# valerio98-lab/DQL_multirotor_landing

Measured on NVIDIA B200. Metric: env_steps_per_sec_incl_q_updates, higher is better.
Workload: dtype f32

## Files before the change

### dql_multirotor_landing_b200/csrc/env_state.cuh

```cuda
#pragma once
#include "dqlb200_device.cuh"

namespace dql {


constexpr int CELLS = DQLB200_MAX_CELLS;
constexpr uint32_t FULL = 0xFFFFFFFFu;

__device__ __forceinline__ uint4 lds128(unsigned addr) {
  uint4 v;
  asm volatile("ld.shared.v4.u32 {%0, %1, %2, %3}, [%4];" : "=r"(v.x), "=r"(v.y), "=r"(v.z), "=r"(v.w) : "r"(addr) : "memory");
  return v;
}

constexpr uint32_t SID_BITS = 10, STEP_SHIFT = 10, STEP_BITS = 9, CC_SHIFT = 19, CC_BITS = 5;
constexpr uint32_t STICKY_BIT = 1u << 24, FRESH_BIT = 1u << 25, BP_SHIFT = 26;

struct Env {
  Body b;
  uint32_t sp_idx;
  float prev_rel_p, prev_rel_v;
  uint32_t sid, bp, step_count, curriculum_check;
  bool sticky_success, fresh;
  uint32_t episode;
  double cum_reward;
};

constexpr size_t ENV_TILE_BYTES = 3 * 32 * 16;
struct EnvPtrs {
  unsigned char* base;
  int n_p, tiles_per_pop;
  uint4* d;
  uint4* e;
  size_t n;
  const double* sp_value;
  const uint2* sp_next;
  const double* sp_rtheta;
  int sp_zero, n_sp;
};
__device__ __forceinline__ unsigned char* env_addr(const EnvPtrs& p, int pop, int env) {
  return p.base + ((size_t)pop * p.tiles_per_pop + (size_t)(env >> 5)) * ENV_TILE_BYTES + (size_t)(env & 31) * 16;
}
__device__ __forceinline__ unsigned char* env_addr(const EnvPtrs& p, size_t i) {
  const int pop = (int)(i / (size_t)p.n_p);
  return env_addr(p, pop, (int)(i - (size_t)pop * p.n_p));
}
__device__ __forceinline__ Ext ext_load(const EnvPtrs& p, size_t i) {
  const uint4 u = p.e[i], v = p.e[p.n + i];
  return Ext{__uint_as_float(u.x), __uint_as_float(u.y), __uint_as_float(u.z), __uint_as_float(u.w),
             __uint_as_float(v.x), __uint_as_float(v.y), __uint_as_float(v.z), __uint_as_float(v.w)};
}
__device__ __forceinline__ void ext_store(const EnvPtrs& p, size_t i, const Ext& x) {
  p.e[i] = make_uint4(__float_as_uint(x.omega), __float_as_uint(x.z), __float_as_uint(x.v_z), __float_as_uint(x.integ));
  p.e[p.n + i] = make_uint4(__float_as_uint(x.e1), __float_as_uint(x.f1), __float_as_uint(x.f2), __float_as_uint(x.f3));
}
template <class KT>
__device__ __forceinline__ Ext ext_initial(const KT& kc) { return Ext{0.0f, kc.z_init, 0.0f, kc.pid_i0, 0.0f, 0.0f, 0.0f, 0.0f}; }
__device__ __forceinline__ Kf kf_load(const EnvPtrs& p, size_t i) {
  const uint4 v = p.d[i];
  return Kf{__uint_as_float(v.x), __uint_as_float(v.y), __uint_as_float(v.z), v.w};
}
__device__ __forceinline__ void kf_store(const EnvPtrs& p, size_t i, const Kf& f) {
  p.d[i] = make_uint4(__float_as_uint(f.x), __float_as_uint(f.P), __float_as_uint(f.v_ref), f.n);
}
__device__ __forceinline__ void ext_prefetch_async(const EnvPtrs& p, size_t i, unsigned stage_addr, int nt, bool filt, bool so) {
  if (filt) asm volatile("cp.async.cg.shared.global [%0], [%1], 16;" ::"r"(stage_addr), "l"(p.d + i) : "memory");
  if (so) {
    asm volatile("cp.async.cg.shared.global [%0], [%1], 16;" ::"r"(stage_addr + 16u * nt), "l"(p.e + i) : "memory");
    asm volatile("cp.async.cg.shared.global [%0], [%1], 16;" ::"r"(stage_addr + 32u * nt), "l"(p.e + p.n + i) : "memory");
  }
  asm volatile("cp.async.commit_group;" ::: "memory");
}
__device__ __forceinline__ Kf kf_take(unsigned stage_addr, int nt) {
  asm volatile("cp.async.wait_group 0;" ::: "memory");
  const uint4 v = lds128(stage_addr);
  return Kf{__uint_as_float(v.x), __uint_as_float(v.y), __uint_as_float(v.z), v.w};
}
__device__ __forceinline__ Ext ext_take(unsigned stage_addr, int nt) {
  asm volatile("cp.async.wait_group 0;" ::: "memory");
  const uint4 u = lds128(stage_addr + 16u * nt), v = lds128(stage_addr + 32u * nt);
  return Ext{__uint_as_float(u.x), __uint_as_float(u.y), __uint_as_float(u.z), __uint_as_float(u.w),
             __uint_as_float(v.x), __uint_as_float(v.y), __uint_as_float(v.z), __uint_as_float(v.w)};
}
__device__ __forceinline__ Kf kf_initial() { return Kf{0.0f, 1.0f, 0.0f, 0u}; }

struct EnvRaw {
  float4 A;
  uint4 B, C;
};
__device__ __forceinline__ EnvRaw env_fetch(const unsigned char* pa) {
  EnvRaw r;
  r.A = __ldcg(reinterpret_cast<const float4*>(pa));
  r.B = __ldcg(reinterpret_cast<const uint4*>(pa + 512));
  r.C = __ldcg(reinterpret_cast<const uint4*>(pa + 1024));
  return r;
}
__device__ __forceinline__ void tile_mbar_init(unsigned mbar) {
  asm volatile("mbarrier.init.shared::cta.b64 [%0], 1;" ::"r"(mbar) : "memory");
  asm volatile("fence.mbarrier_init.release.cluster;" ::: "memory");
  asm volatile("fence.proxy.async.shared::cta;" ::: "memory");
}
__device__ __forceinline__ void tile_prefetch_bulk(const unsigned char* tile, unsigned stage_tile, unsigned mbar) {
  asm volatile("mbarrier.arrive.expect_tx.shared::cta.b64 _, [%0], %1;" ::"r"(mbar), "n"((int)ENV_TILE_BYTES) : "memory");
  asm volatile("cp.async.bulk.shared::cluster.global.mbarrier::complete_tx::bytes [%0], [%1], %2, [%3];" ::"r"(stage_tile), "l"(tile),
               "n"((int)ENV_TILE_BYTES), "r"(mbar)
               : "memory");
}
__device__ __forceinline__ void tile_wait(unsigned mbar, uint32_t parity) {
  asm volatile(
      "{\n"
      ".reg .pred p;\n"
      "TILE_WAIT:\n"
      "mbarrier.try_wait.parity.shared::cta.b64 p, [%0], %1;\n"
      "@p bra TILE_DONE;\n"
      "bra TILE_WAIT;\n"
      "TILE_DONE:\n"
      "}\n" ::"r"(mbar),
      "r"(parity)
      : "memory");
}
__device__ __forceinline__ EnvRaw tile_take(unsigned stage_lane) {
  EnvRaw r;
  const uint4 a = lds128(stage_lane);
  r.A = make_float4(__uint_as_float(a.x), __uint_as_float(a.y), __uint_as_float(a.z), __uint_as_float(a.w));
  r.B = lds128(stage_lane + 512u);
  r.C = lds128(stage_lane + 1024u);
  return r;
}

__device__ __forceinline__ void env_unpack(const EnvRaw& r, Env& e) {
  const float4 A = r.A;
  const uint4 B = r.B;
  const uint4 Cw = r.C;
  e.b.x_d = A.x; e.b.v_d = A.y; e.b.theta = A.z; e.b.phase = __float_as_uint(A.w); e.b.a_d = 0.0f;
  e.sp_idx = B.x;
  e.prev_rel_p = __uint_as_float(B.z);
  e.prev_rel_v = __uint_as_float(B.w);
  e.sid = Cw.x & ((1u << SID_BITS) - 1u);
  e.step_count = (Cw.x >> STEP_SHIFT) & ((1u << STEP_BITS) - 1u);
  e.curriculum_check = (Cw.x >> CC_SHIFT) & ((1u << CC_BITS) - 1u);
  e.sticky_success = (Cw.x & STICKY_BIT) != 0u;
  e.bp = (Cw.x >> BP_SHIFT) & 3u;
  e.fresh = (Cw.x & FRESH_BIT) != 0u;
  e.episode = Cw.y;
  e.cum_reward = __hiloint2double((int)Cw.w, (int)Cw.z);
}
__device__ __forceinline__ void env_store(unsigned char* pa, const Env& e) {
  __stcg(reinterpret_cast<float4*>(pa), make_float4(e.b.x_d, e.b.v_d, e.b.theta, __uint_as_float(e.b.phase)));
  __stcg(reinterpret_cast<uint4*>(pa + 512), make_uint4(e.sp_idx, 0u, __float_as_uint(e.prev_rel_p), __float_as_uint(e.prev_rel_v)));
  const uint32_t packed = e.sid | (e.step_count << STEP_SHIFT) | (e.curriculum_check << CC_SHIFT) |
                          (e.sticky_success ? STICKY_BIT : 0u) | (e.fresh ? FRESH_BIT : 0u) | (e.bp << BP_SHIFT);
  __stcg(reinterpret_cast<uint4*>(pa + 1024), make_uint4(packed, e.episode, (uint32_t)__double2loint(e.cum_reward),
                                                          (uint32_t)__double2hiint(e.cum_reward)));
}
__device__ __forceinline__ void env_load(const EnvPtrs& p, size_t i, Env& e) { env_unpack(env_fetch(env_addr(p, i)), e); }
__device__ __forceinline__ void env_store(const EnvPtrs& p, size_t i, const Env& e) { env_store(env_addr(p, i), e); }

template <class KT, class AC>
__device__ __forceinline__ void env_reset(const KT& kc, const dqlb200_population_params& pp,
                                          const dqlb200_cuts& cuts, const AC& angle_cut, Env& e,
                                          uint32_t env_index, uint32_t birth, int w, bool fresh_mdp, uint32_t sp_zero, Kf* kf = nullptr, Ext* ext = nullptr) {
  const uint4 d = philox4x32_10(make_uint4(env_index, birth, PURPOSE_RESET, pp.population_id), pp.seed_lo, pp.seed_hi);
  Obs o = dyn_reset(kc, pp, e.b, d, w == 0, false, kc.dz_train, kf, ext);
  if (kc.noise_enabled) {
    const uint4 dn = philox4x32_10(make_uint4(env_index, birth, PURPOSE_RESET_NOISE, pp.population_id), pp.seed_lo, pp.seed_hi);
    add_observation_noise(kc, o, dn.x, dn.y);
  }
  const DState ds0 = discretise_cuts(cuts, angle_cut, o);
  e.sid = (uint32_t)ds0.id();
  e.bp = (uint32_t)ds0.bp;
  e.step_count = 0;
  e.curriculum_check = 0;
  e.sticky_success = false;
  e.fresh = true;
  e.cum_reward = 0.0;
  if (fresh_mdp) {
    e.sp_idx = sp_zero;
    e.prev_rel_p = 0.0f;
    e.prev_rel_v = 0.0f;
    e.episode = 0;
  }
}


}
```

### dql_multirotor_landing_b200/csrc/train_kernel.cuh

```cuda
#pragma once
#include <type_traits>

#include "env_state.cuh"

namespace dql {

#define DQL_BAR_CASE(OP, ID) case (ID - 1): if (WARPS >= ID) asm volatile("barrier." OP " " #ID ", 64;" ::: "memory"); break;
template <int WARPS>
__device__ __forceinline__ void baton_wait(int warp) {
  switch (warp) {
    DQL_BAR_CASE("sync", 1) DQL_BAR_CASE("sync", 2) DQL_BAR_CASE("sync", 3) DQL_BAR_CASE("sync", 4)
    DQL_BAR_CASE("sync", 5) DQL_BAR_CASE("sync", 6) DQL_BAR_CASE("sync", 7) DQL_BAR_CASE("sync", 8)
    default: break;
  }
}
template <int WARPS>
__device__ __forceinline__ void baton_pass(int next_warp) {
  switch (next_warp) {
    DQL_BAR_CASE("arrive", 1) DQL_BAR_CASE("arrive", 2) DQL_BAR_CASE("arrive", 3) DQL_BAR_CASE("arrive", 4)
    DQL_BAR_CASE("arrive", 5) DQL_BAR_CASE("arrive", 6) DQL_BAR_CASE("arrive", 7) DQL_BAR_CASE("arrive", 8)
    default: break;
  }
}
#undef DQL_BAR_CASE

#ifdef DQL_TIMING
__device__ unsigned long long dql_timing[4096 * 8];
#define DQL_STAMP(i)                                                                                                      \
  do {                                                                                                                    \
    if (threadIdx.x == 0 && blockIdx.x < 2048) {                                                                          \
      unsigned long long t_;                                                                                              \
      asm volatile("mov.u64 %0, %%globaltimer;" : "=l"(t_)::"memory");                                                    \
      dql_timing[blockIdx.x * 8 + (i)] = t_;                                                                              \
    }                                                                                                                     \
  } while (0)
#else
#define DQL_STAMP(i) do { } while (0)
#endif

struct TrainArgs {
  EnvPtrs env;
  uint32_t* tables;
  dqlb200_population_state* pop_state;
  const dqlb200_population_params* pop_params;
  const float* alpha_luts;
  const uint32_t* eps_threshold;
  dqlb200_trace trace;
  uint32_t* merge_snapshot;
  int k_steps;
  int pop_offset;
  long long n_total;
};

constexpr int RESET_QUEUE = 64;

constexpr int STATES = DQLB200_MAX_CURRICULUM * DQLB200_STATES_PER_LEVEL;

constexpr int EP_OK_CAP = 128;
constexpr int EP_RET_CAP = 32;

struct Shared {
  float qa[CELLS];
  uint32_t cnt[CELLS];
  float qmax[STATES];
  uint8_t greedy[STATES + 3];
  dqlb200_cuts cuts;
  dqlb200_reward_level reward[DQLB200_MAX_CURRICULUM];
  dqlb200_population_state ps;
  uint32_t step_episodes, step_success, step_ep_steps, step_hist[9];
  int promote, advance, do_advance;
  uint4 philox_keys[5];
  double ep_ret[EP_RET_CAP];
  uint8_t ep_ok[EP_OK_CAP];
  int n_ep_ok, n_ep_ret;
};

struct SpEntry {
  uint32_t next;
  float value;
  double r_step, r_first;
};
__host__ __device__ constexpr size_t train_sp_bytes(int n_setpoints) { return ((size_t)n_setpoints * 3 * sizeof(SpEntry) + 15) & ~size_t(15); }
__host__ __device__ constexpr size_t train_smem_bytes(int threads, bool extended, int n_setpoints) {
  return ((sizeof(Shared) + 15) & ~size_t(15)) + train_sp_bytes(n_setpoints) + (size_t)(threads / 32) * RESET_QUEUE * sizeof(uint16_t) +
         (size_t)(extended ? 6 : 3) * threads * 16 + (((size_t)(threads / 32) * 8 + 15) & ~size_t(15));
}

static_assert((train_smem_bytes(128, false, 33) + 1024) * 6 <= 228 * 1024, "train_kernel<4>: six CTAs per SM no longer fit in shared memory");
#ifndef DQL_WARPS_PER_SM
#define DQL_WARPS_PER_SM 24
#endif
#ifndef DQL_WARPS_PER_SM_GENERIC
#define DQL_WARPS_PER_SM_GENERIC 20
#endif
template <bool GENERIC_> struct ConstsOf;
template <> struct ConstsOf<true> {
  __device__ __forceinline__ static const KC& get(const KC& kc) { return kc; }
};
template <> struct ConstsOf<false> {
  __device__ __forceinline__ static KDef get(const KC&) { return KDef{}; }
};

template <int WARPS, bool TRACE, int VARIANT>
__global__ void __launch_bounds__(WARPS * 32, ((VARIANT == 2 ? DQL_WARPS_PER_SM_GENERIC : DQL_WARPS_PER_SM) / WARPS) > 0 ? ((VARIANT == 2 ? DQL_WARPS_PER_SM_GENERIC : DQL_WARPS_PER_SM) / WARPS) : 1) train_kernel(const __grid_constant__ KC kc, const TrainArgs args) {
  constexpr bool GENERIC = VARIANT == 1 || VARIANT == 2, EXT = VARIANT == 2, FULL_SLOTS = VARIANT == 3;
  extern __shared__ __align__(16) unsigned char smem_raw[];
  Shared& sh = *reinterpret_cast<Shared*>(smem_raw);
  DQL_STAMP(0);
#ifdef DQL_TIMING
  if (threadIdx.x == 0 && blockIdx.x < 2048) {
    unsigned smid_, warpid_;
    asm volatile("mov.u32 %0, %%smid;" : "=r"(smid_));
    asm volatile("mov.u32 %0, %%warpid;" : "=r"(warpid_));
    dql_timing[4096 * 8 - 1 - blockIdx.x] = ((unsigned long long)smid_ << 32) | warpid_;
  }
#endif
  const auto& kk = ConstsOf<GENERIC>::get(kc);
  const int tid = threadIdx.x, lane = tid & 31, warp = tid >> 5;
  constexpr int NT = WARPS * 32;
  const int pop = blockIdx.x + args.pop_offset;
  const int n_p = kc.envs_per_population;
  const int n_slots = (n_p + NT - 1) / NT;
  unsigned char* dyn = smem_raw + ((sizeof(Shared) + 15) & ~size_t(15));
  uint16_t* reset_queue = reinterpret_cast<uint16_t*>(dyn) + (size_t)warp * RESET_QUEUE;
  dyn += (size_t)WARPS * RESET_QUEUE * sizeof(uint16_t);
  uint4* stage = reinterpret_cast<uint4*>(dyn);
  dyn += (size_t)((TRACE || EXT) ? 6 : 3) * NT * 16;
  unsigned long long* tile_mbar = reinterpret_cast<unsigned long long*>(dyn);
  dyn += ((size_t)WARPS * 8 + 15) & ~size_t(15);
  SpEntry* sp_tab = reinterpret_cast<SpEntry*>(dyn);
  const unsigned stage_tile = (unsigned)__cvta_generic_to_shared(stage) + (unsigned)warp * (unsigned)ENV_TILE_BYTES;
  const unsigned stage_lane = stage_tile + (unsigned)lane * 16u;
  const unsigned ext_stage = (unsigned)__cvta_generic_to_shared(stage + WARPS * 96 + tid);
  const unsigned mbar = (unsigned)__cvta_generic_to_shared(tile_mbar + warp);
  const int tiles_pp = args.env.tiles_per_pop;
  uint32_t tile_phase = 0u;
  bool tile_pending = false;
  auto prefetch_tile = [&](const unsigned char* tile) {
    __syncwarp();
    if (lane == 0) tile_prefetch_bulk(tile, stage_tile, mbar);
    tile_pending = true;
  };
  auto env_writes_done = [&]() { asm volatile("fence.proxy.async.global;" ::: "memory"); };
  auto wait_tile = [&]() {
    tile_wait(mbar, tile_phase);
    tile_phase ^= 1u;
    tile_pending = false;
  };
  const size_t env_base = (size_t)pop * n_p;
  uint32_t* gt = args.tables + (size_t)pop * 3 * CELLS;
  float* gqb = reinterpret_cast<float*>(gt + CELLS);
  const uint32_t sp_zero = (uint32_t)args.env.sp_zero;

  static_assert(sizeof(dqlb200_population_state) % 4 == 0, "word copies");
  constexpr int PS_WORDS = sizeof(dqlb200_population_state) / 4;
  const dqlb200_population_params pp = args.pop_params[pop];
  unsigned char* const p_tile0 = env_addr(args.env, pop, warp * 32);
  if (lane == 0) tile_mbar_init(mbar);
  if (warp < tiles_pp) prefetch_tile(p_tile0);
  if (EXT) ext_prefetch_async(args.env, env_base + (size_t)min(tid, n_p - 1), ext_stage, NT, kc.accel_mode != 0, kc.dynamics_model != 0);
  {
    const int w_start = args.pop_state[pop].working_step;
    const uint32_t* gps = reinterpret_cast<const uint32_t*>(args.pop_state + pop);
    for (int i = tid; i < PS_WORDS; i += NT) reinterpret_cast<uint32_t*>(&sh.ps)[i] = gps[i];
    if (tid == 0) {
      sh.step_episodes = sh.step_success = sh.step_ep_steps = 0u;
      for (int i = 0; i < 9; ++i) sh.step_hist[i] = 0u;
      sh.promote = sh.advance = sh.do_advance = 0;
      sh.n_ep_ok = sh.n_ep_ret = 0;
      sh.cuts = kc.cuts[w_start];
    }
    if (tid < 5) sh.reward[tid] = kc.reward[tid];
    if (tid == 31) philox_round_keys(pp.seed_lo, pp.seed_hi, sh.philox_keys);
    for (int i = tid; i < args.env.n_sp * 3; i += NT) {
      const uint2 nx = args.env.sp_next[i];
      sp_tab[i] = SpEntry{nx.x, __uint_as_float(nx.y), args.env.sp_rtheta[i], args.env.sp_rtheta[DQLB200_MAX_SETPOINTS * 3 + i]};
    }
    const int live = (w_start + 1) * DQLB200_CELLS_PER_LEVEL;
    for (int i = tid; i < DQLB200_CELLS_PER_LEVEL; i += NT) {
      sh.qa[i] = __uint_as_float(gt[i]);
      sh.cnt[i] = gt[2 * CELLS + i];
      if ((i & 31) == 0) asm volatile("prefetch.global.L2 [%0];" ::"l"(gqb + i));
    }
    for (int i = DQLB200_CELLS_PER_LEVEL + tid; i < live; i += NT) {
      sh.qa[i] = __uint_as_float(gt[i]);
      sh.cnt[i] = gt[2 * CELLS + i];
      if ((i & 31) == 0) asm volatile("prefetch.global.L2 [%0];" ::"l"(gqb + i));
    }
  }
  __syncthreads();

  DQL_STAMP(1);
  const float* __restrict__ alpha_lut = args.alpha_luts + (size_t)pp.alpha_lut * DQLB200_ALPHA_LUT;
  const float alpha_min = __ldg(alpha_lut + DQLB200_ALPHA_LUT - 1);
  const bool filt = EXT && kc.accel_mode != 0;
  const bool so = EXT && kc.dynamics_model != 0;
  uint64_t steps_done = 0;

  auto build_snapshot = [&](int w) {
    for (int st = tid; st < (w + 1) * DQLB200_STATES_PER_LEVEL; st += NT) {
      const float q0 = sh.qa[st * 3 + 0], q1 = sh.qa[st * 3 + 1], q2 = sh.qa[st * 3 + 2];
      const float p0 = fmul(fadd(q0, __ldcg(gqb + st * 3 + 0)), 0.5f);
      const float p1 = fmul(fadd(q1, __ldcg(gqb + st * 3 + 1)), 0.5f);
      const float p2 = fmul(fadd(q2, __ldcg(gqb + st * 3 + 2)), 0.5f);
      int a = 0;
      float best = p0;
      if (p1 > best) { best = p1; a = 1; }
      if (p2 > best) { a = 2; }
      sh.greedy[st] = (uint8_t)a;
      sh.qmax[st] = fmaxf(fmaxf(q0, q1), q2);
    }
  };

  auto drain_episode_log = [&]() {
    dqlb200_population_state& ps = sh.ps;
    const int n_fin = sh.n_ep_ok, n_ret = sh.n_ep_ret;
    if (n_fin == 0) return;
    const int L = kc.window_len;
    bool promote = false;
    if (lane == 31) {
      double s = ps.return_sum;
      for (int i = 0; i < n_ret; ++i) s = __dadd_rn(s, sh.ep_ret[i]);
      ps.return_sum = s;
    }
    for (int base = 0; base < n_fin; base += 32) {
      const int n = min(32, n_fin - base);
      const bool mine = lane < n;
      const int ok = mine ? (int)sh.ep_ok[base + lane] : 0;
      const uint32_t smask = __ballot_sync(FULL, ok != 0);
      const int head = ps.window_head, count = ps.window_count, sum = ps.window_sum;
      if (n <= L) {
        int pos = head + lane;
        pos -= (pos >= L) ? L : 0;
        const bool evicts = mine && (count + lane >= L);
        const int old = evicts ? (int)ps.window[pos] : 0;
        const uint32_t emask = __ballot_sync(FULL, evicts && old != 0);
        const uint32_t upto = (2u << lane) - 1u;
        const int s_here = sum + __popc(smask & upto) - __popc(emask & upto);
        promote = promote || __any_sync(FULL, mine && s_here >= kc.promote_successes);
        __syncwarp();
        if (mine) ps.window[pos] = (uint8_t)ok;
        if (lane == 0) {
          int h2 = head + n;
          h2 -= (h2 >= L) ? L : 0;
          ps.window_head = h2;
          ps.window_count = min(count + n, L);
          ps.window_sum = sum + __popc(smask) - __popc(emask);
        }
      } else {
        bool pr = false;
        if (lane == 0) {
          int h2 = head, c2 = count, s2 = sum;
          for (int b = 0; b < n; ++b) {
            const int okb = (smask >> b) & 1u;
            if (c2 == L) s2 -= ps.window[h2];
            else c2 += 1;
            ps.window[h2] = (uint8_t)okb;
            s2 += okb;
            h2 = (h2 + 1 == L) ? 0 : h2 + 1;
            pr = pr || (s2 >= kc.promote_successes);
          }
          ps.window_head = h2; ps.window_count = c2; ps.window_sum = s2;
        }
        promote = promote || (__shfl_sync(FULL, (int)pr, 0) != 0);
      }
      __syncwarp();
    }
    if (lane == 0) {
      ps.episodes_in_step += n_fin;
      if (kc.replicas == 1) {
        if (promote) sh.promote = 1;
        if (ps.episodes_in_step >= kc.max_num_episodes) sh.advance = 1;
      }
      sh.n_ep_ok = sh.n_ep_ret = 0;
    }
    __syncwarp();
  };

  auto advance_curriculum = [&](int w, uint32_t birth) {
    const int cs = kc.curriculum_steps;
    int dst = -1, src = 0;
    float ratio = 1.0f;
    if (kc.transfer_mode == 0) { dst = w; src = (w - 1 + cs) % cs; ratio = kc.transfer_ratio[w]; }
    else if (w + 1 < cs) { dst = w + 1; src = w; ratio = kc.transfer_ratio[w + 1]; }
    if (dst >= 0) {
      uint32_t* sg = (args.merge_snapshot && pop % kc.replicas == 0) ? args.merge_snapshot + (size_t)(pop / kc.replicas) * 3 * CELLS : nullptr;
      for (int i = tid; i < DQLB200_CELLS_PER_LEVEL; i += NT) {
        const float q_src = (src <= w) ? sh.qa[src * DQLB200_CELLS_PER_LEVEL + i] : __uint_as_float(gt[src * DQLB200_CELLS_PER_LEVEL + i]);
        const float qa_new = fmul(q_src, ratio), qb_new = fmul(gqb[src * DQLB200_CELLS_PER_LEVEL + i], ratio);
        sh.qa[dst * DQLB200_CELLS_PER_LEVEL + i] = qa_new;
        gqb[dst * DQLB200_CELLS_PER_LEVEL + i] = qb_new;
        if (sg) {
          sg[dst * DQLB200_CELLS_PER_LEVEL + i] = __float_as_uint(qa_new);
          sg[CELLS + dst * DQLB200_CELLS_PER_LEVEL + i] = __float_as_uint(qb_new);
        }
      }
    }
    if (w + 1 < cs) {
      for (int i = tid; i < DQLB200_CELLS_PER_LEVEL; i += NT) {
        const int c = (w + 1) * DQLB200_CELLS_PER_LEVEL + i;
        if (dst != w + 1) sh.qa[c] = __uint_as_float(gt[c]);
        sh.cnt[c] = gt[2 * CELLS + c];
      }
    }
    __syncthreads();
    if (tid == 0) {
      dqlb200_population_state& ps = sh.ps;
      if (sh.promote) { ps.window_head = ps.window_count = ps.window_sum = 0; }
      ps.promoted_at[w] = birth;
      ps.episodes_in_step = 0;
      ps.pending_advance = 0;
      sh.promote = sh.advance = sh.do_advance = 0;
      if (w + 1 >= cs) ps.finished = 1;
      else {
        ps.working_step = w + 1;
        sh.cuts = kc.cuts[w + 1];
      }
    }
    __syncthreads();
    if (!sh.ps.finished) {
      for (int slot = 0; slot < n_slots; ++slot) {
        const int env_i = slot * NT + tid;
        if (env_i < n_p) {
          Env e;
          Kf kf;
          Ext ex;
          if (filt) kf = kf_load(args.env, env_base + env_i);
          if (so) ex = ext_load(args.env, env_base + env_i);
          env_reset(kk, pp, sh.cuts, kk.angle_cut, e, (uint32_t)env_i, birth, w + 1, true, sp_zero, filt ? &kf : nullptr, so ? &ex : nullptr);
          env_store(env_addr(args.env, pop, env_i), e);
          if (filt) kf_store(args.env, env_base + env_i, kf);
          if (so) ext_store(args.env, env_base + env_i, ex);
        }
      }
      env_writes_done();
      if (tile_pending) wait_tile();
      if (warp < tiles_pp) prefetch_tile(p_tile0);
      if (EXT) {
        asm volatile("cp.async.wait_group 0;" ::: "memory");
        ext_prefetch_async(args.env, env_base + (size_t)min(tid, n_p - 1), ext_stage, NT, filt, so);
      }
      build_snapshot(w + 1);
    }
    __syncthreads();
  };
  if (sh.ps.pending_advance && !sh.ps.finished) {
    if (tid == 0) sh.promote = (sh.ps.pending_advance == 1) ? 1 : 0;
    __syncthreads();
    advance_curriculum(sh.ps.working_step, sh.ps.t);
  } else {
    build_snapshot(sh.ps.working_step);
    __syncthreads();
  }

  DQL_STAMP(2);
  for (int k = 0; k < args.k_steps; ++k) {
    if (sh.ps.finished) break;
    const int w = sh.ps.working_step;
    const uint32_t t = sh.ps.t;
    int n_queued = 0;

    auto flush_resets = [&]() {
      __syncwarp();
      for (int base = 0; base < n_queued; base += 32) {
        if (base + lane < n_queued) {
          const int qv = reset_queue[base + lane];
          const int env_r = (qv >> 5) * NT + warp * 32 + (qv & 31);
          const size_t gr = env_base + (size_t)env_r;
          unsigned char* const pr = env_addr(args.env, pop, env_r);
          Env e;
          env_unpack(env_fetch(pr), e);
          Kf kf;
          Ext ex;
          if (filt) kf = kf_load(args.env, gr);
          if (so) ex = ext_load(args.env, gr);
          env_reset(kk, pp, sh.cuts, kk.angle_cut, e, (uint32_t)env_r, t + 1u, w, false, sp_zero, filt ? &kf : nullptr, so ? &ex : nullptr);
          env_store(pr, e);
          if (filt) kf_store(args.env, gr, kf);
          if (so) ext_store(args.env, gr, ex);
        }
      }
      __syncwarp();
      n_queued = 0;
    };

    auto slot_loop = [&](auto w0_tag) {
    constexpr bool W0 = decltype(w0_tag)::value;
    bool bad_obs = false;
    unsigned char* p_env = env_addr(args.env, pop, tid);
    for (int slot = 0; slot < n_slots; ++slot) {
      const int env_i = slot * NT + tid;
      const bool valid = FULL_SLOTS || env_i < n_p;
      const size_t gi = env_base + (size_t)env_i;
      if (FULL_SLOTS || slot * WARPS + warp < tiles_pp) wait_tile();
      if (slot == 0) DQL_STAMP(7);
      const EnvRaw cur_raw = tile_take(stage_lane);
      unsigned char* const p_cur = p_env;
      p_env += WARPS * ENV_TILE_BYTES;
      Kf kf;
      Ext ex;
      if (filt) kf = kf_take(ext_stage, NT);
      if (so) ex = ext_take(ext_stage, NT);
      if (FULL_SLOTS ? (slot + 1 < n_slots) : ((slot + 1) * WARPS + warp < tiles_pp)) prefetch_tile(p_env - (size_t)lane * 16);
      if (EXT && env_i + NT < n_p) ext_prefetch_async(args.env, gi + NT, ext_stage, NT, filt, so);
      uint32_t cell = 0;
      float target = 0.0f;
      bool done = false, success = false;
      int code = 0;
      uint32_t ep_steps = 0;
      double ep_return = 0.0;
      Env e;
      int a = 0;
      uint32_t sid = 0u, noise_w0 = 0u, noise_w1 = 0u;
      size_t trace_i = 0;
      if (valid) {
        env_unpack(cur_raw, e);
        sid = e.sid;
        a = sh.greedy[sid];
        if (W0 || w == 0 || (GENERIC && kk.noise_enabled)) {
          const uint4 d = philox4x32_10_keyed(make_uint4((uint32_t)env_i, t, PURPOSE_STEP, pp.population_id), sh.philox_keys);
          if (W0 || w == 0) {
            const uint32_t thr = __ldg(args.eps_threshold + min(e.episode, (uint32_t)(DQLB200_EPS_LUT - 1)));
            if ((d.x >> 8) < thr) a = (int)__umulhi(d.y, 3u);
          }
          if (GENERIC) { noise_w0 = d.z; noise_w1 = d.w; }
        }
        if (TRACE) {
          trace_i = (size_t)k * (size_t)args.n_total + gi;
          if (args.trace.action_override) {
            const int o = args.trace.action_override[trace_i];
            if (o >= 0) a = o;
          }
        }
        cell = sid * 3u + (uint32_t)a;
      }
      uint32_t peers;
      asm volatile("match.any.sync.b32 %0, %1, 0xffffffff;" : "=r"(peers) : "r"(valid ? cell : (0x80000000u | (uint32_t)lane)) : "memory");
      uint2 spn = make_uint2(0u, 0u);
      double r_theta0 = 0.0;
      Obs o = {};
      DState ds = {};
      uint32_t sid2 = 0u, step_count = 0u, cc = 0u;
      if (valid) {
        const uint32_t sp_prev = e.sp_idx;
        {
          const SpEntry* en = sp_tab + (e.fresh ? sp_zero : sp_prev) * 3u + (uint32_t)a;
          spn = make_uint2(en->next, __float_as_uint(en->value));
        }
        const float sp = __uint_as_float(spn.y);
        r_theta0 = *(&sp_tab[sp_prev * 3u + (uint32_t)a].r_step + (e.fresh ? 1 : 0));
        dyn_advance(kk, pp, e.b, sp, filt ? &kf : nullptr, so ? &ex : nullptr, kk.vz_train);
        step_count = e.step_count + 1u;
        o = dyn_observe(kk, pp, e.b, (int)step_count, kk.dz_train, filt ? &kf : nullptr, so ? &ex : nullptr);
        if (GENERIC && kk.noise_enabled) add_observation_noise(kk, o, noise_w0, noise_w1);
        ds = W0 ? discretise_cuts(kc.cuts[0], kk.angle_cut, o, 0) : discretise_cuts(sh.cuts, kk.angle_cut, o, w);
        sid2 = (uint32_t)ds.id();
        const bool t_fx = !(o.rel_p >= kk.fz_lo) || (o.rel_p >= kk.fz_hi);
        const bool t_zmin = !(o.z >= kk.z_min_cut), t_zmax = o.z >= kk.z_max_cut;
        const bool t_time = (int)step_count >= kk.timeout_steps;
        const bool goal_bins = !(o.contact || t_fx || t_zmin || t_zmax || t_time) && ds.bp == 1 && ds.bv == 1;
        const bool at_level = W0 || (sid >= (uint32_t)(w * DQLB200_STATES_PER_LEVEL) && ds.level == w);
        cc = goal_bins ? (at_level ? e.curriculum_check + 1u : 0u) : e.curriculum_check;
        code = e.sticky_success ? DQLB200_NON_TERMINAL_SUCCESS : DQLB200_NON_TERMINAL;
        if (goal_bins && at_level) code = ((int)cc >= kk.success_steps) ? DQLB200_TERMINAL_SUCCESS : DQLB200_NON_TERMINAL_SUCCESS;
        code = t_time ? DQLB200_TERMINAL_TIMEOUT : code;
        code = t_zmax ? DQLB200_TERMINAL_FLYZONE_Z : code;
        code = t_zmin ? DQLB200_TERMINAL_MINIMUM_ALTITUDE : code;
        code = t_fx ? DQLB200_TERMINAL_FLYZONE_X : code;
        code = o.contact ? DQLB200_TERMINAL_CONTACT : code;
        done = code >= DQLB200_TERMINAL_SUCCESS;
        success = code == DQLB200_TERMINAL_SUCCESS;
        bad_obs = bad_obs || !(fabsf(o.rel_p) <= 3.4028234664e38f) || !(fabsf(o.rel_v) <= 3.4028234664e38f) || !(fabsf(o.rel_a) <= 3.4028234664e38f);
      }
      const uint32_t lower = peers & ((1u << lane) - 1u);
      const int rank = __popc(lower);
      const int n_group = valid ? __popc(peers) : 0;
      const int pred = lower ? (31 - __clz(lower)) : lane;
      const bool is_last = valid && (peers >> lane) == 1u;
      const int n_max = __reduce_max_sync(FULL, n_group);
      const uint32_t c_hint = min(sh.cnt[cell] + (uint32_t)rank, (uint32_t)(DQLB200_ALPHA_LUT - 1));
      const float a_hint = __ldg(alpha_lut + c_hint);
      if (valid) {
        const double phi_p = shaping(kk.w_p, o.rel_p, kk.p_max, kk.rcp_p_max, kk.clip_p_f, GENERIC);
        const double phi_v = shaping(kk.w_v, o.rel_v, kk.v_max, kk.rcp_v_max, kk.clip_v_f, GENERIC);
        const double prev_p = shaping(kk.w_p, e.prev_rel_p, kk.p_max, kk.rcp_p_max, kk.clip_p_f, GENERIC);
        const double prev_v = shaping(kk.w_v, e.prev_rel_v, kk.v_max, kk.rcp_v_max, kk.clip_v_f, GENERIC);
        const bool succ_reward = code == DQLB200_NON_TERMINAL_SUCCESS || code == DQLB200_TERMINAL_SUCCESS;
        const double r = reward_sp(W0 ? kc.reward[0] : sh.reward[ds.level], phi_p, phi_v, prev_p, prev_v, r_theta0, succ_reward);
        const float qn = sh.qmax[sid2];
        const float changed = (e.bp != (uint32_t)ds.bp) ? 1.0f : 0.0f;
        target = fadd((float)r, fmul(fmul(kk.gamma, qn), changed));
        if (TRACE) {
          if (args.trace.obs) {
            float* po = args.trace.obs + trace_i * 5;
            po[0] = o.rel_p; po[1] = o.rel_v; po[2] = o.rel_a; po[3] = o.pitch; po[4] = o.z;
          }
          if (args.trace.reward) args.trace.reward[trace_i] = r;
          if (args.trace.action) args.trace.action[trace_i] = (uint8_t)a;
          if (args.trace.code) args.trace.code[trace_i] = (uint8_t)code;
          if (args.trace.done) args.trace.done[trace_i] = (uint8_t)done;
          if (args.trace.contact) args.trace.contact[trace_i] = (uint8_t)o.contact;
          if (args.trace.state) args.trace.state[trace_i] = (uint16_t)sid;
          if (args.trace.next_state) args.trace.next_state[trace_i] = (uint16_t)sid2;
          if (args.trace.episode) args.trace.episode[trace_i] = (int32_t)e.episode;
        }
        ep_steps = step_count;
        ep_return = e.cum_reward;
        e.sp_idx = spn.x;
        e.prev_rel_p = o.rel_p;
        e.prev_rel_v = o.rel_v;
        e.episode += done ? 1u : 0u;
        e.sid = sid2;
        e.bp = (uint32_t)ds.bp;
        e.step_count = step_count;
        e.curriculum_check = cc;
        e.sticky_success = (code == DQLB200_NON_TERMINAL_SUCCESS);
        e.fresh = false;
        e.cum_reward = __dadd_rn(e.cum_reward, r);
      }
      const uint32_t dmask = __ballot_sync(FULL, valid && done);
      uint32_t smask = 0u;
      double ret = 0.0;
      if (dmask) {
        smask = __ballot_sync(FULL, valid && success);
        ret = (valid && done) ? ep_return : 0.0;
#pragma unroll
        for (int off = 16; off > 0; off >>= 1) ret = __dadd_rn(ret, __shfl_xor_sync(FULL, ret, off));
      }
      if (WARPS > 1 && !(slot == 0 && warp == 0)) baton_wait<WARPS>(warp);
      {
        float q = sh.qa[cell];
        const uint32_t c0 = sh.cnt[cell];
        const uint32_t c_pre = min(c0 + (uint32_t)rank, (uint32_t)(DQLB200_ALPHA_LUT - 1));
        float alpha = a_hint;
        if (c_pre != c_hint) alpha = __ldg(alpha_lut + c_pre);
        if (rank == 0) q = fadd(q, fmul(alpha, fsub(target, q)));
#pragma unroll 1
        for (int r = 1; r < n_max; ++r) {
          const float qp = __shfl_sync(FULL, q, pred);
          if (rank == r) q = fadd(qp, fmul(alpha, fsub(target, qp)));
        }
        if (is_last) {
          sh.qa[cell] = q;
          sh.cnt[cell] = c0 + (uint32_t)n_group;
        }
        if (dmask) {
          if (sh.n_ep_ret == EP_RET_CAP || sh.n_ep_ok > EP_OK_CAP - 32) drain_episode_log();
          const int idx = sh.n_ep_ret, base = sh.n_ep_ok;
          const int last = 31 - __clz(dmask);
          __syncwarp();
          if (valid && done) sh.ep_ok[base + __popc(dmask & ((1u << lane) - 1u))] = (uint8_t)success;
          if (lane == 0) {
            sh.ep_ret[idx] = ret;
            sh.n_ep_ret = idx + 1;
            sh.n_ep_ok = base + __popc(dmask);
          }
          if (lane == last) {
            sh.ps.last_cumulative = ep_return;
            sh.ps.last_steps = (int)ep_steps;
            sh.ps.last_code = code;
          }
        }
      }
      if (WARPS > 1 && !(slot == n_slots - 1 && warp == WARPS - 1)) {
        baton_pass<WARPS>((warp + 1) % WARPS);
      }
      if (dmask) {
        if (valid && done) {
          atomicAdd(&sh.step_hist[code], 1u);
          atomicAdd(&sh.step_ep_steps, ep_steps);
        }
        if (lane == 0) {
          atomicAdd(&sh.step_episodes, (uint32_t)__popc(dmask));
          atomicAdd(&sh.step_success, (uint32_t)__popc(smask));
        }
      }
      if (valid) env_store(p_cur, e);
      if (filt && valid) kf_store(args.env, gi, kf);
      if (so && valid) ext_store(args.env, gi, ex);
      if (dmask) {
        if (valid && done) reset_queue[n_queued + __popc(dmask & ((1u << lane) - 1u))] = (uint16_t)(slot * 32 + lane);
        n_queued += __popc(dmask);
        if (n_queued > RESET_QUEUE - 32) flush_resets();
      }
      if (slot == 0) DQL_STAMP(6);
    }
    if (bad_obs) atomicOr(&sh.ps.error_flags, 1u);
    };
    if constexpr (!GENERIC && !TRACE) {
      if (w == 0) slot_loop(std::true_type{});
      else slot_loop(std::false_type{});
    } else {
      slot_loop(std::false_type{});
    }
    flush_resets();
    env_writes_done();
    if (k + 1 < args.k_steps) {
      if (warp < tiles_pp) prefetch_tile(p_tile0);
      if (EXT) ext_prefetch_async(args.env, env_base + (size_t)min(tid, n_p - 1), ext_stage, NT, filt, so);
    }
    __syncthreads();
    DQL_STAMP(3);
    steps_done += (uint64_t)n_p;
    if (warp == 0) drain_episode_log();
    if (tid == 0) {
      sh.ps.t = t + 1u;
      sh.do_advance = (sh.promote || sh.advance) ? 1 : 0;
      sh.ps.total_episodes += sh.step_episodes; sh.ps.total_successes += sh.step_success; sh.ps.episode_steps_sum += sh.step_ep_steps;
      sh.step_episodes = sh.step_success = sh.step_ep_steps = 0u;
    }
    if (tid < 9) { sh.ps.termination_hist[tid] += sh.step_hist[tid]; sh.step_hist[tid] = 0u; }
    if (k + 1 < args.k_steps) build_snapshot(w);
    __syncthreads();
    if (sh.do_advance) advance_curriculum(w, t + 1u);
  }

  DQL_STAMP(4);
  if (tile_pending) wait_tile();
  if (EXT) asm volatile("cp.async.wait_all;" ::: "memory");
  for (int i = tid; i < (sh.ps.working_step + 1) * DQLB200_CELLS_PER_LEVEL; i += NT) {
    gt[i] = __float_as_uint(sh.qa[i]);
    gt[2 * CELLS + i] = sh.cnt[i];
  }
  if (warp == 0) {
    if (lane == 0) {
      dqlb200_population_state& ps = sh.ps;
      ps.total_steps += steps_done;
    }
    __syncwarp();
    uint32_t* gps = reinterpret_cast<uint32_t*>(args.pop_state + pop);
    for (int i = lane; i < PS_WORDS; i += 32) gps[i] = reinterpret_cast<const uint32_t*>(&sh.ps)[i];
  }
  DQL_STAMP(5);
}


}
```

Baseline: 28.95 billion.

## Pair consecutive env tiles per warp in stage-0 loop to halve baton handoffs

In the w==0 fast path, each warp now processes two adjacent env tiles per baton turn. The front half of the first tile is stashed in idle rows of the Q-table shared memory, and a second bulk tile prefetch lands in that scratch area. Both Q-updates are then committed under a single baton wait/pass, cutting the serialized inter-warp handoffs in half. Reset-queue indexing and tile addressing are remapped to the paired layout. The cost is more complex mbarrier expect_tx/arrive bookkeeping, reliance on unused shared table rows, and extra register/stash traffic.

```diff
diff --git a/dql_multirotor_landing_b200/csrc/env_state.cuh b/dql_multirotor_landing_b200/csrc/env_state.cuh
--- a/dql_multirotor_landing_b200/csrc/env_state.cuh
+++ b/dql_multirotor_landing_b200/csrc/env_state.cuh
@@ -106,6 +106,13 @@
                "n"((int)ENV_TILE_BYTES), "r"(mbar)
                : "memory");
 }
+__device__ __forceinline__ void tile_prefetch_bulk_noarrive(const unsigned char* tile, unsigned stage_tile, unsigned mbar) {
+  asm volatile("mbarrier.expect_tx.relaxed.cta.shared::cta.b64 [%0], %1;" ::"r"(mbar), "n"((int)ENV_TILE_BYTES) : "memory");
+  asm volatile("cp.async.bulk.shared::cluster.global.mbarrier::complete_tx::bytes [%0], [%1], %2, [%3];" ::"r"(stage_tile), "l"(tile),
+               "n"((int)ENV_TILE_BYTES), "r"(mbar)
+               : "memory");
+}
+__device__ __forceinline__ void tile_arrive(unsigned mbar) { asm volatile("mbarrier.arrive.shared::cta.b64 _, [%0];" ::"r"(mbar) : "memory"); }
 __device__ __forceinline__ void tile_wait(unsigned mbar, uint32_t parity) {
   asm volatile(
       "{\n"
diff --git a/dql_multirotor_landing_b200/csrc/train_kernel.cuh b/dql_multirotor_landing_b200/csrc/train_kernel.cuh
--- a/dql_multirotor_landing_b200/csrc/train_kernel.cuh
+++ b/dql_multirotor_landing_b200/csrc/train_kernel.cuh
@@ -1,4 +1,5 @@
 #pragma once
+#include <cstddef>
 #include <type_traits>
 
 #include "env_state.cuh"
@@ -85,6 +86,33 @@
   return ((sizeof(Shared) + 15) & ~size_t(15)) + train_sp_bytes(n_setpoints) + (size_t)(threads / 32) * RESET_QUEUE * sizeof(uint16_t) +
          (size_t)(extended ? 6 : 3) * threads * 16 + (((size_t)(threads / 32) * 8 + 15) & ~size_t(15));
 }
+
+struct PairStash {
+  uint4 lane[32];
+  uint32_t dmask, smask, n_max, last_sc;
+  double ret, last_ret;
+};
+constexpr size_t PAIR_QA = (DQLB200_CELLS_PER_LEVEL * sizeof(float) + 15) & ~size_t(15);
+constexpr size_t PAIR_CNT = (offsetof(Shared, cnt) + DQLB200_CELLS_PER_LEVEL * sizeof(uint32_t) + 15) & ~size_t(15);
+constexpr size_t PAIR_QA_END = offsetof(Shared, qa) + CELLS * sizeof(float), PAIR_CNT_END = offsetof(Shared, cnt) + CELLS * sizeof(uint32_t);
+constexpr int PAIR_TILES_IN_QA = (int)((PAIR_QA_END - PAIR_QA) / ENV_TILE_BYTES);
+__host__ __device__ constexpr size_t pair_tile_off(int warp) {
+  return warp < PAIR_TILES_IN_QA ? PAIR_QA + (size_t)warp * ENV_TILE_BYTES : PAIR_CNT + (size_t)(warp - PAIR_TILES_IN_QA) * ENV_TILE_BYTES;
+}
+__host__ __device__ constexpr size_t pair_stash_off(int warps, int warp) {
+  return PAIR_CNT + (size_t)(warps > PAIR_TILES_IN_QA ? warps - PAIR_TILES_IN_QA : 0) * ENV_TILE_BYTES + (size_t)warp * sizeof(PairStash);
+}
+static_assert(offsetof(Shared, qa) == 0 && sizeof(PairStash) % 16 == 0, "scratch offsets are 16-byte aligned");
+static_assert(PAIR_TILES_IN_QA >= 4 && pair_stash_off(8, 8) <= PAIR_CNT_END, "paired slots: second tiles and stashes of 8 warps no longer fit in the idle table rows");
+
+struct TileFront {
+  Env e;
+  uint32_t cell, c_hint, ep_steps, dmask, smask;
+  float target, a_hint;
+  int code, rank, pred, n_group, n_max;
+  bool done, is_last;
+  double ep_return, ret;
+};
 
 static_assert((train_smem_bytes(128, false, 33) + 1024) * 6 <= 228 * 1024, "train_kernel<4>: six CTAs per SM no longer fit in shared memory");
 #ifndef DQL_WARPS_PER_SM
@@ -155,12 +183,13 @@
   static_assert(sizeof(dqlb200_population_state) % 4 == 0, "word copies");
   constexpr int PS_WORDS = sizeof(dqlb200_population_state) / 4;
   const dqlb200_population_params pp = args.pop_params[pop];
-  unsigned char* const p_tile0 = env_addr(args.env, pop, warp * 32);
+  constexpr bool PAIRED_W0 = FULL_SLOTS && !GENERIC && !TRACE;
+  auto tile0 = [&](int w_) { return env_addr(args.env, pop, ((PAIRED_W0 && w_ == 0 && n_slots > 1) ? 2 * warp : warp) * 32); };
+  const int w_start = args.pop_state[pop].working_step;
   if (lane == 0) tile_mbar_init(mbar);
-  if (warp < tiles_pp) prefetch_tile(p_tile0);
+  if (warp < tiles_pp) prefetch_tile(tile0(w_start));
   if (EXT) ext_prefetch_async(args.env, env_base + (size_t)min(tid, n_p - 1), ext_stage, NT, kc.accel_mode != 0, kc.dynamics_model != 0);
   {
-    const int w_start = args.pop_state[pop].working_step;
     const uint32_t* gps = reinterpret_cast<const uint32_t*>(args.pop_state + pop);
     for (int i = tid; i < PS_WORDS; i += NT) reinterpret_cast<uint32_t*>(&sh.ps)[i] = gps[i];
     if (tid == 0) {
@@ -335,7 +364,7 @@
       }
       env_writes_done();
       if (tile_pending) wait_tile();
-      if (warp < tiles_pp) prefetch_tile(p_tile0);
+      if (warp < tiles_pp) prefetch_tile(tile0(w + 1));
       if (EXT) {
         asm volatile("cp.async.wait_group 0;" ::: "memory");
         ext_prefetch_async(args.env, env_base + (size_t)min(tid, n_p - 1), ext_stage, NT, filt, so);
@@ -360,12 +389,15 @@
     const uint32_t t = sh.ps.t;
     int n_queued = 0;
 
-    auto flush_resets = [&]() {
+    auto flush_resets = [&](auto paired_tag) {
+      constexpr bool PAIRED = decltype(paired_tag)::value;
       __syncwarp();
       for (int base = 0; base < n_queued; base += 32) {
         if (base + lane < n_queued) {
           const int qv = reset_queue[base + lane];
-          const int env_r = (qv >> 5) * NT + warp * 32 + (qv & 31);
+          const int j = qv >> 5;
+          const int env_r = (PAIRED && ((j & 1) || j + 1 < n_slots)) ? (j & ~1) * NT + (2 * warp + (j & 1)) * 32 + (qv & 31)
+                                                                      : j * NT + warp * 32 + (qv & 31);
           const size_t gr = env_base + (size_t)env_r;
           unsigned char* const pr = env_addr(args.env, pop, env_r);
           Env e;
@@ -384,32 +416,15 @@
       n_queued = 0;
     };
 
-    auto slot_loop = [&](auto w0_tag) {
-    constexpr bool W0 = decltype(w0_tag)::value;
-    bool bad_obs = false;
-    unsigned char* p_env = env_addr(args.env, pop, tid);
-    for (int slot = 0; slot < n_slots; ++slot) {
-      const int env_i = slot * NT + tid;
-      const bool valid = FULL_SLOTS || env_i < n_p;
-      const size_t gi = env_base + (size_t)env_i;
-      if (FULL_SLOTS || slot * WARPS + warp < tiles_pp) wait_tile();
-      if (slot == 0) DQL_STAMP(7);
-      const EnvRaw cur_raw = tile_take(stage_lane);
-      unsigned char* const p_cur = p_env;
-      p_env += WARPS * ENV_TILE_BYTES;
-      Kf kf;
-      Ext ex;
-      if (filt) kf = kf_take(ext_stage, NT);
-      if (so) ex = ext_take(ext_stage, NT);
-      if (FULL_SLOTS ? (slot + 1 < n_slots) : ((slot + 1) * WARPS + warp < tiles_pp)) prefetch_tile(p_env - (size_t)lane * 16);
-      if (EXT && env_i + NT < n_p) ext_prefetch_async(args.env, gi + NT, ext_stage, NT, filt, so);
+    auto tile_front = [&](auto w0_tag, TileFront& f, const EnvRaw& cur_raw, int env_i, bool valid, size_t gi, Kf& kf, Ext& ex, bool& bad_obs) {
+      constexpr bool W0 = decltype(w0_tag)::value;
       uint32_t cell = 0;
       float target = 0.0f;
       bool done = false, success = false;
       int code = 0;
       uint32_t ep_steps = 0;
       double ep_return = 0.0;
-      Env e;
+      Env& e = f.e;
       int a = 0;
       uint32_t sid = 0u, noise_w0 = 0u, noise_w1 = 0u;
       size_t trace_i = 0;
@@ -527,76 +542,172 @@
 #pragma unroll
         for (int off = 16; off > 0; off >>= 1) ret = __dadd_rn(ret, __shfl_xor_sync(FULL, ret, off));
       }
+      f.cell = cell; f.c_hint = c_hint; f.ep_steps = ep_steps; f.dmask = dmask; f.smask = smask;
+      f.target = target; f.a_hint = a_hint;
+      f.code = code; f.rank = rank; f.pred = pred; f.n_group = n_group; f.n_max = n_max;
+      f.done = done; f.is_last = is_last;
+      f.ep_return = ep_return; f.ret = ret;
+    };
+
+    auto tile_commit = [&](uint32_t cell, float target, float a_hint, uint32_t c_hint, int rank, int pred, int n_group, bool is_last, int n_max,
+                           uint32_t dmask, uint32_t smask, double ret, int writer, double last_ret, uint32_t last_steps, int last_code, bool done, bool success) {
+      float q = sh.qa[cell];
+      const uint32_t c0 = sh.cnt[cell];
+      const uint32_t c_pre = min(c0 + (uint32_t)rank, (uint32_t)(DQLB200_ALPHA_LUT - 1));
+      float alpha = a_hint;
+      if (c_pre != c_hint) alpha = __ldg(alpha_lut + c_pre);
+      if (rank == 0) q = fadd(q, fmul(alpha, fsub(target, q)));
+#pragma unroll 1
+      for (int r = 1; r < n_max; ++r) {
+        const float qp = __shfl_sync(FULL, q, pred);
+        if (rank == r) q = fadd(qp, fmul(alpha, fsub(target, qp)));
+      }
+      if (is_last) {
+        sh.qa[cell] = q;
+        sh.cnt[cell] = c0 + (uint32_t)n_group;
+      }
+      if (dmask) {
+        if (sh.n_ep_ret == EP_RET_CAP || sh.n_ep_ok > EP_OK_CAP - 32) drain_episode_log();
+        const int idx = sh.n_ep_ret, base = sh.n_ep_ok;
+        const int last = writer >= 0 ? writer : 31 - __clz(dmask);
+        __syncwarp();
+        if (done) sh.ep_ok[base + __popc(dmask & ((1u << lane) - 1u))] = (uint8_t)success;
+        if (lane == 0) {
+          sh.ep_ret[idx] = ret;
+          sh.n_ep_ret = idx + 1;
+          sh.n_ep_ok = base + __popc(dmask);
+        }
+        if (lane == last) {
+          sh.ps.last_cumulative = last_ret;
+          sh.ps.last_steps = (int)last_steps;
+          sh.ps.last_code = last_code;
+        }
+      }
+    };
+
+    auto tile_back = [&](auto paired_tag, const TileFront& f, unsigned char* p_cur, bool valid, size_t gi, const Kf& kf, const Ext& ex, int j) {
+      if (f.dmask) {
+        if (valid && f.done) {
+          atomicAdd(&sh.step_hist[f.code], 1u);
+          atomicAdd(&sh.step_ep_steps, f.ep_steps);
+        }
+        if (lane == 0) {
+          atomicAdd(&sh.step_episodes, (uint32_t)__popc(f.dmask));
+          atomicAdd(&sh.step_success, (uint32_t)__popc(f.smask));
+        }
+      }
+      if (valid) env_store(p_cur, f.e);
+      if (filt && valid) kf_store(args.env, gi, kf);
+      if (so && valid) ext_store(args.env, gi, ex);
+      if (f.dmask) {
+        if (valid && f.done) reset_queue[n_queued + __popc(f.dmask & ((1u << lane) - 1u))] = (uint16_t)(j * 32 + lane);
+        n_queued += __popc(f.dmask);
+        if (n_queued > RESET_QUEUE - 32) flush_resets(paired_tag);
+      }
+    };
+
+    auto slot_loop = [&](auto w0_tag) {
+    bool bad_obs = false;
+    unsigned char* p_env = env_addr(args.env, pop, tid);
+    for (int slot = 0; slot < n_slots; ++slot) {
+      const int env_i = slot * NT + tid;
+      const bool valid = FULL_SLOTS || env_i < n_p;
+      const size_t gi = env_base + (size_t)env_i;
+      if (FULL_SLOTS || slot * WARPS + warp < tiles_pp) wait_tile();
+      if (slot == 0) DQL_STAMP(7);
+      const EnvRaw cur_raw = tile_take(stage_lane);
+      unsigned char* const p_cur = p_env;
+      p_env += WARPS * ENV_TILE_BYTES;
+      Kf kf;
+      Ext ex;
+      if (filt) kf = kf_take(ext_stage, NT);
+      if (so) ex = ext_take(ext_stage, NT);
+      if (FULL_SLOTS ? (slot + 1 < n_slots) : ((slot + 1) * WARPS + warp < tiles_pp)) prefetch_tile(p_env - (size_t)lane * 16);
+      if (EXT && env_i + NT < n_p) ext_prefetch_async(args.env, gi + NT, ext_stage, NT, filt, so);
+      TileFront f;
+      tile_front(w0_tag, f, cur_raw, env_i, valid, gi, kf, ex, bad_obs);
       if (WARPS > 1 && !(slot == 0 && warp == 0)) baton_wait<WARPS>(warp);
-      {
-        float q = sh.qa[cell];
-        const uint32_t c0 = sh.cnt[cell];
-        const uint32_t c_pre = min(c0 + (uint32_t)rank, (uint32_t)(DQLB200_ALPHA_LUT - 1));
-        float alpha = a_hint;
-        if (c_pre != c_hint) alpha = __ldg(alpha_lut + c_pre);
-        if (rank == 0) q = fadd(q, fmul(alpha, fsub(target, q)));
-#pragma unroll 1
-        for (int r = 1; r < n_max; ++r) {
-          const float qp = __shfl_sync(FULL, q, pred);
-          if (rank == r) q = fadd(qp, fmul(alpha, fsub(target, qp)));
-        }
-        if (is_last) {
-          sh.qa[cell] = q;
-          sh.cnt[cell] = c0 + (uint32_t)n_group;
-        }
-        if (dmask) {
-          if (sh.n_ep_ret == EP_RET_CAP || sh.n_ep_ok > EP_OK_CAP - 32) drain_episode_log();
-          const int idx = sh.n_ep_ret, base = sh.n_ep_ok;
-          const int last = 31 - __clz(dmask);
-          __syncwarp();
-          if (valid && done) sh.ep_ok[base + __popc(dmask & ((1u << lane) - 1u))] = (uint8_t)success;
-          if (lane == 0) {
-            sh.ep_ret[idx] = ret;
-            sh.n_ep_ret = idx + 1;
-            sh.n_ep_ok = base + __popc(dmask);
-          }
-          if (lane == last) {
-            sh.ps.last_cumulative = ep_return;
-            sh.ps.last_steps = (int)ep_steps;
-            sh.ps.last_code = code;
-          }
-        }
-      }
+      tile_commit(f.cell, f.target, f.a_hint, f.c_hint, f.rank, f.pred, f.n_group, f.is_last, f.n_max, f.dmask, f.smask, f.ret, -1, f.ep_return, f.ep_steps, f.code,
+                  valid && f.done, valid && f.code == DQLB200_TERMINAL_SUCCESS);
       if (WARPS > 1 && !(slot == n_slots - 1 && warp == WARPS - 1)) {
         baton_pass<WARPS>((warp + 1) % WARPS);
       }
-      if (dmask) {
-        if (valid && done) {
-          atomicAdd(&sh.step_hist[code], 1u);
-          atomicAdd(&sh.step_ep_steps, ep_steps);
-        }
-        if (lane == 0) {
-          atomicAdd(&sh.step_episodes, (uint32_t)__popc(dmask));
-          atomicAdd(&sh.step_success, (uint32_t)__popc(smask));
-        }
-      }
-      if (valid) env_store(p_cur, e);
-      if (filt && valid) kf_store(args.env, gi, kf);
-      if (so && valid) ext_store(args.env, gi, ex);
-      if (dmask) {
-        if (valid && done) reset_queue[n_queued + __popc(dmask & ((1u << lane) - 1u))] = (uint16_t)(slot * 32 + lane);
-        n_queued += __popc(dmask);
-        if (n_queued > RESET_QUEUE - 32) flush_resets();
-      }
+      tile_back(std::false_type{}, f, p_cur, valid, gi, kf, ex, slot);
       if (slot == 0) DQL_STAMP(6);
     }
     if (bad_obs) atomicOr(&sh.ps.error_flags, 1u);
+    flush_resets(std::false_type{});
     };
-    if constexpr (!GENERIC && !TRACE) {
+
+    auto paired_loop = [&]() {
+      bool bad_obs = false;
+      const int n_super = (n_slots + 1) >> 1;
+      unsigned char* const pop_tiles = env_addr(args.env, pop, 0);
+      const unsigned scratch_tile = (unsigned)__cvta_generic_to_shared(smem_raw) + (unsigned)pair_tile_off(warp);
+      PairStash& st = *reinterpret_cast<PairStash*>(smem_raw + pair_stash_off(WARPS, warp));
+      Kf kf;
+      Ext ex;
+      for (int s = 0; s < n_super; ++s) {
+        const bool pair = 2 * s + 1 < n_slots, more = s + 1 < n_super, pair_next = 2 * s + 3 < n_slots;
+        const int ta = pair ? 2 * (s * WARPS + warp) : 2 * s * WARPS + warp;
+        const int tn = pair_next ? 2 * ((s + 1) * WARPS + warp) : 2 * (s + 1) * WARPS + warp;
+        const int nh = pair ? 2 : 1;
+#pragma unroll 1
+        for (int h = 0; h < nh; ++h) {
+          if (h == 0 || s == 0) wait_tile();
+          if (s == 0 && h == 0) DQL_STAMP(7);
+          const EnvRaw raw = tile_take((h ? scratch_tile : stage_tile) + (unsigned)lane * 16u);
+          __syncwarp();
+          if (lane == 0) {
+            if (h == 0) {
+              if (more) tile_prefetch_bulk_noarrive(pop_tiles + (size_t)tn * ENV_TILE_BYTES, stage_tile, mbar);
+              if (s == 0 && pair) tile_prefetch_bulk(pop_tiles + (size_t)(ta + 1) * ENV_TILE_BYTES, scratch_tile, mbar);
+            } else if (more) {
+              if (pair_next) tile_prefetch_bulk(pop_tiles + (size_t)(tn + 1) * ENV_TILE_BYTES, scratch_tile, mbar);
+              else tile_arrive(mbar);
+            }
+          }
+          const int env_i = (ta + h) * 32 + lane;
+          TileFront f;
+          tile_front(std::true_type{}, f, raw, env_i, true, env_base + (size_t)env_i, kf, ex, bad_obs);
+          if (h + 1 < nh) {
+            st.lane[lane] = make_uint4(__float_as_uint(f.target), __float_as_uint(f.a_hint),
+                                       f.cell | (uint32_t)f.rank << 12 | (uint32_t)f.pred << 17 | (uint32_t)f.n_group << 22 | (uint32_t)f.is_last << 28, f.c_hint);
+            if (lane == 0) { st.dmask = f.dmask; st.smask = f.smask; st.n_max = (uint32_t)f.n_max; st.ret = f.ret; }
+            if (f.dmask && lane == 31 - __clz(f.dmask)) { st.last_sc = f.ep_steps | (uint32_t)f.code << 16; st.last_ret = f.ep_return; }
+          } else {
+            if (WARPS > 1 && !(s == 0 && warp == 0)) baton_wait<WARPS>(warp);
+            if (h == 1) {
+              __syncwarp();
+              const uint4 sl = st.lane[lane];
+              tile_commit(sl.z & 0xFFFu, __uint_as_float(sl.x), __uint_as_float(sl.y), sl.w, (int)((sl.z >> 12) & 31u), (int)((sl.z >> 17) & 31u),
+                          (int)((sl.z >> 22) & 63u), ((sl.z >> 28) & 1u) != 0u, (int)st.n_max, st.dmask, st.smask, st.ret, 0, st.last_ret,
+                          st.last_sc & 0xFFFFu, (int)(st.last_sc >> 16), ((st.dmask >> lane) & 1u) != 0u,
+                          ((st.smask >> lane) & 1u) != 0u);
+            }
+            tile_commit(f.cell, f.target, f.a_hint, f.c_hint, f.rank, f.pred, f.n_group, f.is_last, f.n_max, f.dmask, f.smask, f.ret, -1, f.ep_return, f.ep_steps, f.code,
+                        f.done, f.code == DQLB200_TERMINAL_SUCCESS);
+            if (WARPS > 1 && !(s == n_super - 1 && warp == WARPS - 1)) baton_pass<WARPS>((warp + 1) % WARPS);
+          }
+          tile_back(std::true_type{}, f, pop_tiles + (size_t)(ta + h) * ENV_TILE_BYTES + (size_t)lane * 16, true, 0, kf, ex, 2 * s + h);
+        }
+        if (s == 0) DQL_STAMP(6);
+      }
+      if (bad_obs) atomicOr(&sh.ps.error_flags, 1u);
+      flush_resets(std::true_type{});
+    };
+    if constexpr (PAIRED_W0) {
+      if (w == 0) paired_loop();
+      else slot_loop(std::false_type{});
+    } else if constexpr (!GENERIC && !TRACE) {
       if (w == 0) slot_loop(std::true_type{});
       else slot_loop(std::false_type{});
     } else {
       slot_loop(std::false_type{});
     }
-    flush_resets();
     env_writes_done();
     if (k + 1 < args.k_steps) {
-      if (warp < tiles_pp) prefetch_tile(p_tile0);
+      if (warp < tiles_pp) prefetch_tile(tile0(w));
       if (EXT) ext_prefetch_async(args.env, env_base + (size_t)min(tid, n_p - 1), ext_stage, NT, filt, so);
     }
     __syncthreads();
```

Measured after the change: 24.47 billion, median of 6. -15.5%, worse.
